# kingdwd/nlp-filter

Measured on AMD Instinct MI355X. Metric: Gauss-Newton collocation-point updates/sec, higher is better.
Workload: dtype f64; 1 GPU; C2 van_der_pol: n=2, m=1, full_state p=2, N=100 (P=101, d=202), T=10, M=101; global_batch=1024, batch_per_gpu=1024, parallelism=dp1 (independent trajectories; RCCL broadcast of constants only)

## Files before the change

### nlp-filter_amd/csrc/mhe_core.h

```cpp
#pragma once
#include <hip/hip_runtime.h>
#include <math.h>
#include <mutex>
#include <stdint.h>
#include <stdlib.h>

#include "mhe.h"
#include "mhe_models.h"

namespace mhe {

typedef double d4 __attribute__((ext_vector_type(4)));

#ifndef MHE_GN_MINW
#define MHE_GN_MINW 4
#endif
#ifndef MHE_NW
#define MHE_NW 8
#endif
constexpr int NW = MHE_NW;
constexpr int NTHREADS = NW * 64;
constexpr int MAX_NT = 13;
constexpr int MAX_SLOTS = (MAX_NT * (MAX_NT - 1) / 2 + NW - 1) / NW;

// ... 67 lines not shown
  S.ROWM = o; o += NW * 8;
  S.UN = o;   o += UNITS;
  S.XO = o;   o += bounded ? rnd2(P * n) : 0;
  S.ACT = o;  o += bounded ? dp / 2 : 0;
  S.GV = o;   o += bounded ? dp : 0;
  S.ZP = o;   o += cov ? dp * 16 : 0;
  S.total = o;
  return S;
}

struct GnArgs {
  const char* cbuf;
  int P, M, d, NT, ntiles, q, has_prior;
  int idx[8];
  double alpha;
  const double* X0;
  double* Xout;
  const double* U;
  long long ustride;
  const double* Y;
  const double* PAR;
  long long pstride;
  const double* x0;
  double* cost;
  int* iters;
  int* status;
  int max_iter;
  double tol;
  double* Hout;
  double* gout;
  const double* Hin;
  const double* gin;
  double* dout;
  unsigned long long* dbg;
  double huber_delta;
  int n_bounds;
  unsigned long long tag;
  int bidx[8];
  double blb[8], bub[8];
  double dpar[8];
  const double* Rw;
  long long rwstride;
  const double* PhiQ;
  int nq;
  double* cov;
  const double* md;
  long long mdstride;
  const double* Pw;
  long long pwstride;
  const double* Z0;
  double* Zout;
  double* lam;
  int nz, nc;
};

__device__ __forceinline__ const double* prior_weight(const GnArgs& a, const ConstLayout& CL, int b) {
  return a.Pw ? a.Pw + (long long)b * a.pwstride : (const double*)(a.cbuf + CL.Pw);
}

#ifdef MHE_DIAG
#define DIAG_DECL unsigned long long _dg[16] = {}; unsigned long long _dt = __builtin_amdgcn_s_memtime();
#define DIAG_MARK(i) do { const unsigned long long _n = __builtin_amdgcn_s_memtime(); _dg[i] += _n - _dt; _dt = _n; } while (0)
#define DIAG_FLUSH(b) do { if (threadIdx.x == 0 && a.dbg) for (int _i = 0; _i < 16; ++_i) a.dbg[(b) * 16 + _i] = _dg[_i]; } while (0)
#define DIAG_FDECL unsigned long long* _dg, unsigned long long& _dt
#define DIAG_FARGS _dg, _dt
#else
#define DIAG_DECL
#define DIAG_MARK(i) do { } while (0)
#define DIAG_FLUSH(b) do { } while (0)
#define DIAG_FDECL int
#define DIAG_FARGS 0
#endif

#ifndef MHE_KO
#define MHE_KO 0
#endif
#define KO(bit) ((MHE_KO >> (bit)) & 1)

__device__ __forceinline__ double readlane_d(double v, int lane) {
  const long long b = __double_as_longlong(v);
  const int lo = __builtin_amdgcn_readlane((int)b, lane);
  const int hi = __builtin_amdgcn_readlane((int)(b >> 32), lane);
  return __longlong_as_double(((long long)hi << 32) | (unsigned int)lo);
}

typedef unsigned int mhe_u2 __attribute__((ext_vector_type(2)));
__device__ __forceinline__ __amdgpu_buffer_rsrc_t cbuf_rsrc(const char* cbuf, size_t bytes) {
  return __builtin_amdgcn_make_buffer_rsrc((void*)cbuf, (short)0, (int)bytes, 0x00020000);
}
__device__ __forceinline__ double bload(__amdgpu_buffer_rsrc_t r, int voff, int soff) {
  const mhe_u2 v = __builtin_amdgcn_raw_buffer_load_b64(r, voff, soff, 0);
  return __builtin_bit_cast(double, v);
}

template <int CTRL>
__device__ __forceinline__ double dpp_d(double v) {
  const long long b = __double_as_longlong(v);
  const int lo = __builtin_amdgcn_mov_dpp((int)b, CTRL, 0xF, 0xF, false);
  const int hi = __builtin_amdgcn_mov_dpp((int)(b >> 32), CTRL, 0xF, 0xF, false);
  return __longlong_as_double(((long long)hi << 32) | (unsigned int)lo);
}

__device__ __forceinline__ void spread_dblock(double v, double (&o)[4]) {
  const double ev = dpp_d<0xA0>(v);
  const double od = dpp_d<0xF5>(v);
  const long long be = __double_as_longlong(ev), bo = __double_as_longlong(od);
  const auto el = __builtin_amdgcn_permlane16_swap((int)be, (int)be, false, false);
  const auto eh = __builtin_amdgcn_permlane16_swap((int)(be >> 32), (int)(be >> 32), false, false);
  const auto ol = __builtin_amdgcn_permlane16_swap((int)bo, (int)bo, false, false);
  const auto oh = __builtin_amdgcn_permlane16_swap((int)(bo >> 32), (int)(bo >> 32), false, false);
  o[0] = __longlong_as_double(((long long)eh[0] << 32) | (unsigned int)el[0]);
  o[2] = __longlong_as_double(((long long)eh[1] << 32) | (unsigned int)el[1]);
  o[1] = __longlong_as_double(((long long)oh[0] << 32) | (unsigned int)ol[0]);
  o[3] = __longlong_as_double(((long long)oh[1] << 32) | (unsigned int)ol[1]);
}

template <int XOR16, bool MAX>
__device__ __forceinline__ double pair_combine(double v) {
  const long long b = __double_as_longlong(v);
  const int lo = (int)b, hi = (int)(b >> 32);
  double x, y;
  if constexpr (XOR16 == 1) {
    auto l = __builtin_amdgcn_permlane16_swap(lo, lo, false, false);
    auto h = __builtin_amdgcn_permlane16_swap(hi, hi, false, false);
    x = __longlong_as_double(((long long)h[0] << 32) | (unsigned int)l[0]);
    y = __longlong_as_double(((long long)h[1] << 32) | (unsigned int)l[1]);
  } else {
    auto l = __builtin_amdgcn_permlane32_swap(lo, lo, false, false);
    auto h = __builtin_amdgcn_permlane32_swap(hi, hi, false, false);
    x = __longlong_as_double(((long long)h[0] << 32) | (unsigned int)l[0]);
    y = __longlong_as_double(((long long)h[1] << 32) | (unsigned int)l[1]);
  }
  return MAX ? fmax(x, y) : x + y;
}

__device__ __forceinline__ double wave_sum(double v) {
  v += dpp_d<0xB1>(v);
  v += dpp_d<0x4E>(v);
  v += dpp_d<0x141>(v);
  v += dpp_d<0x140>(v);
  v = pair_combine<1, false>(v);
  return pair_combine<2, false>(v);
}

__device__ __forceinline__ double wave_max(double v) {
  v = fmax(v, dpp_d<0xB1>(v));
  v = fmax(v, dpp_d<0x4E>(v));
  v = fmax(v, dpp_d<0x141>(v));
  v = fmax(v, dpp_d<0x140>(v));
  v = pair_combine<1, true>(v);
  return pair_combine<2, true>(v);
}

__device__ __forceinline__ void block_reduce2(double* red, double& a, double& b, bool is_max) {
  const int lane = threadIdx.x & 63, wave = threadIdx.x >> 6;
  a = is_max ? wave_max(a) : wave_sum(a);
  b = is_max ? wave_max(b) : wave_sum(b);
  if (lane == 0) {
    red[2 * wave] = a;
    red[2 * wave + 1] = b;
  }
  __syncthreads();
  double ra = red[0], rb = red[1];
#pragma unroll
  for (int w = 1; w < NW; ++w) {
    ra = is_max ? fmax(ra, red[2 * w]) : ra + red[2 * w];
    rb = is_max ? fmax(rb, red[2 * w + 1]) : rb + red[2 * w + 1];
  }
  __syncthreads();
  a = ra;
  b = rb;
}

__device__ __forceinline__ int make_slot_table(int wave, int lane, int NT) {
  const int u = wave + NW * lane;
  if (lane >= MAX_SLOTS || u >= NT * (NT - 1) / 2) return -1;
  int J = 0, base = 0;
  while (u >= base + (NT - 1 - J)) {
    base += NT - 1 - J;
    ++J;
  }
  return (J + 1 + (u - base)) | (J << 16);
}

__device__ __forceinline__ int tile_index(int I, int J, int NT) { return J * NT - J * (J - 1) / 2 + (I - J); }

__device__ __forceinline__ int slot_ij(int stab, int s) { return __builtin_amdgcn_readlane(stab, s); }

__device__ __forceinline__ int slot_start(int j, int wave, int NT) {
  const int base = j * (NT - 1) - j * (j - 1) / 2;
  return base > wave ? (base - wave + NW - 1) / NW : 0;
}

__device__ __forceinline__ void init_units(double* un) {
  if (threadIdx.x < 64)
    for (int e = threadIdx.x; e < UNITS; e += 64) un[e] = (e == 16 || e == 51) ? 1.0 : 0.0;
}

template <int SLOTS = MAX_SLOTS>
__device__ __forceinline__ void init_rowmask(int* rowm, int wave, int lane, int stab) {
  unsigned m = 0;
#pragma unroll
  for (int s = 0; s < SLOTS; ++s) {
    const int IJ = slot_ij(stab, s);
    if (IJ >= 0 && (IJ & 0xffff) == lane) m |= 1u << s;
  }
  if (lane < 16) rowm[wave * 16 + lane] = (int)m;
}

constexpr int TPR = NW >= 8 ? 4 : 2;

__device__ __forceinline__ int opaque_tid() {
  int t = threadIdx.x;
  asm volatile("" : "+v"(t));
  return t;
}

template <int n>
__device__ __forceinline__ void dot_rows_part(const double* __restrict__ Mt, int ld, int row, int len, int part,
                                              const double* __restrict__ Xs, double (&acc)[n]) {
#pragma unroll
  for (int c = 0; c < n; ++c) acc[c] = 0.0;
  int j = part;
#pragma unroll 1
  for (; j + TPR * 7 < len; j += TPR * 8) {
    double m[8];
#pragma unroll
    for (int u = 0; u < 8; ++u) m[u] = Mt[(j + TPR * u) * ld + row];
#pragma unroll
    for (int u = 0; u < 8; ++u)
#pragma unroll
      for (int c = 0; c < n; ++c) acc[c] += m[u] * Xs[(j + TPR * u) * n + c];
  }
  for (; j < len; j += TPR) {
    const double mv = Mt[j * ld + row];
#pragma unroll
    for (int c = 0; c < n; ++c) acc[c] += mv * Xs[j * n + c];
  }
  static_assert(TPR == 4, "quad reductions below assume 4 lanes per row");
#pragma unroll
  for (int c = 0; c < n; ++c) acc[c] += dpp_d<0xB1>(acc[c]);
#pragma unroll
  for (int c = 0; c < n; ++c) acc[c] += dpp_d<0x4E>(acc[c]);
}

template <class DYN, bool HUBER = false>
__device__ __forceinline__ double node_row(const GnArgs& a, const ConstLayout& CL, const SmemLayout& SL, double* sm,
                                           int b, int k, const double (&dx)[DYN::n]) {
  constexpr int n = DYN::n, m = DYN::m;
  const double* cw = (const double*)(a.cbuf + CL.cw);
  const double* Qw = (const double*)(a.cbuf + CL.Qw);
  const double* Xs = sm + SL.Xs;
  double cost = 0.0;
  {
    double xk[n], uk[m > 0 ? m : 1], f[n], F[n * n];
#pragma unroll
    for (int c = 0; c < n; ++c) xk[c] = Xs[k * n + c];
    if (m > 0) {
      const double* U = a.U + (long long)b * a.ustride + (long long)k * m;
#pragma unroll
      for (int c = 0; c < m; ++c) uk[c] = U[c];
    }
    DYN::eval(xk, uk, a.dpar, f, F);
    double W[n], V[n];
#pragma unroll
    for (int c = 0; c < n; ++c) W[c] = a.alpha * dx[c] - f[c];
    const double ck = cw[k];
    double E[n * n];
    if constexpr (HUBER) {
      const double dl = a.huber_delta;
#pragma unroll
      for (int r = 0; r < n; ++r) {
        const double q = Qw[r * n + r];
        const double sr = sqrt(1.0 + W[r] * W[r] / (dl * dl));
        const double lam = ck * (q / sr);
        V[r] = lam * W[r];
        cost += ck * (2.0 * q * dl * dl * (sr - 1.0));
        sm[SL.LAM + k * n + r] = lam;
#pragma unroll
        for (int c = 0; c < n; ++c) E[r * n + c] = lam * F[r * n + c];
      }
    } else {
#pragma unroll
      for (int r = 0; r < n; ++r) {
        double s = 0.0;
#pragma unroll
        for (int c = 0; c < n; ++c) s += Qw[r * n + c] * W[c];
        V[r] = ck * s;
        cost += W[r] * V[r];
      }
#pragma unroll
      for (int r = 0; r < n; ++r)
#pragma unroll
        for (int c = 0; c < n; ++c) {
          double s = 0.0;
#pragma unroll
          for (int t = 0; t < n; ++t) s += Qw[r * n + t] * F[t * n + c];
          E[r * n + c] = ck * s;
        }
    }
    double* Vs = sm + SL.Vs + k * n;
    double* FtV = sm + SL.FtV + k * n;
    double* Es = sm + SL.Es + k * n * n;
    double* FtE = sm + SL.FtE + k * n * n;
#pragma unroll
    for (int r = 0; r < n; ++r) {
      Vs[r] = V[r];
      double s = 0.0;
// ... 12 lines not shown
  }
  return cost;
}

template <class DYN, bool HUBER = false>
__device__ __forceinline__ double node_phase(const GnArgs& a, const ConstLayout& CL, const SmemLayout& SL, double* sm, int b) {
  constexpr int n = DYN::n;
  const double* Dt = (const double*)(a.cbuf + CL.Dt);
  const double* Xs = sm + SL.Xs;
  double cost = 0.0;
  const int tid = opaque_tid();
  const int part = tid % TPR;
  for (int k0 = 0; k0 < a.P; k0 += NTHREADS / TPR) {
    const int k = k0 + tid / TPR;
    const int kk = k < a.P ? k : a.P - 1;
    double dx[n];
    dot_rows_part<n>(Dt, a.P, kk, a.P, part, Xs, dx);
    if (part || k >= a.P) continue;
    cost += node_row<DYN, HUBER>(a, CL, SL, sm, b, k, dx);
  }
  return cost;
}

constexpr double COST_NOISE = 4.0;

template <class DYN, class MEAS, bool NOISE = false, bool MHUBER = false>
__device__ __forceinline__ double meas_row(const GnArgs& a, const ConstLayout& CL, const SmemLayout& SL, double* sm,
                                           int b, int i, const double (&xi)[DYN::n], double* nzp = nullptr) {
  constexpr int n = DYN::n, p = MEAS::p, q = MEAS::q;
  const double* Rw = (const double*)(a.cbuf + CL.Rw);
  double cost = 0.0;
  {
    double par[q > 0 ? q : 1];
    if (q > 0) {
      const double* PR = a.PAR + (long long)b * a.pstride + (long long)i * q;
#pragma unroll
      for (int c = 0; c < q; ++c) par[c] = PR[c];
    }
    const double* R = (!MEAS::LINEAR && a.Rw ? a.Rw + (long long)b * a.rwstride : Rw) + (long long)i * p * p;
    double h[p], H[p * n];
    MEAS::eval(xi, par, a.idx, h, H);
    const double* yi = a.Y + ((long long)b * a.M + i) * p;
    double e[p], Re[p];
#pragma unroll
    for (int r = 0; r < p; ++r) e[r] = yi[r] - h[r];
    const bool masked = masked_row<p>(R);
    if (masked) {
#pragma unroll
      for (int c = 0; c < p * n; ++c) H[c] = 0.0;
#pragma unroll
      for (int r = 0; r < p; ++r) e[r] = 0.0;
    }
    [[maybe_unused]] double lam[p], rcost = 0.0;
    [[maybe_unused]] bool robust = false;
    if constexpr (MHUBER) {
      static_assert(p == 1 && !MEAS::LINEAR, "robust measurement rows: scalar rows of a nonlinear model");
      lam[0] = R[0];
      const double dl = a.md[(long long)b * a.mdstride + i];
      if (!masked && dl < INFINITY) {
        const double sr = sqrt(1.0 + e[0] * e[0] / (dl * dl));
        lam[0] = R[0] / sr;
        rcost = 2.0 * R[0] * e[0] * e[0] / (1.0 + sr);
        robust = true;
      }
      R = lam;
    }
#pragma unroll
    for (int r = 0; r < p; ++r) {
      double s = 0.0;
#pragma unroll
      for (int c = 0; c < p; ++c) s += R[r * p + c] * e[c];
      Re[r] = s;
      cost += e[r] * s;
    }
    if constexpr (MHUBER) {
      if (robust) cost = rcost;
    }
    if constexpr (NOISE) {
      if (!masked) {
        double t = 0.0;
#pragma unroll
        for (int r = 0; r < p; ++r) t += fabs(Re[r]) * (fabs(yi[r]) + fabs(h[r]));
        *nzp += COST_NOISE * __DBL_EPSILON__ * t;
      }
    }
    double* GE = sm + SL.GE + i * n;
#pragma unroll
    for (int c = 0; c < n; ++c) {
      double s = 0.0;
#pragma unroll
      for (int r = 0; r < p; ++r) s += H[r * n + c] * Re[r];
      GE[c] = s;
    }
    if (!MEAS::LINEAR) {
      double* G = sm + SL.G + i * n * n;
      double RH[p * n];
#pragma unroll
      for (int r = 0; r < p; ++r)
#pragma unroll
        for (int c = 0; c < n; ++c) {
          double s = 0.0;
#pragma unroll
          for (int t = 0; t < p; ++t) s += R[r * p + t] * H[t * n + c];
          RH[r * n + c] = s;
        }
#pragma unroll
      for (int r = 0; r < n; ++r)
#pragma unroll
        for (int c = 0; c < n; ++c) {
          double s = 0.0;
#pragma unroll
          for (int t = 0; t < p; ++t) s += H[t * n + r] * RH[t * n + c];
          G[r * n + c] = s;
        }
    }
  }
  return cost;
}

template <class DYN, class MEAS, bool NOISE = false, bool MHUBER = false>
__device__ __forceinline__ double meas_phase(const GnArgs& a, const ConstLayout& CL, const SmemLayout& SL, double* sm, int b,
                                             double* nzp = nullptr) {
  constexpr int n = DYN::n;
  const double* PhiT = (const double*)(a.cbuf + CL.PhiT);
  const double* Xs = sm + SL.Xs;
  double cost = 0.0;
  const int tid = opaque_tid();
  const int part = tid % TPR;
  for (int i0 = 0; i0 < a.M; i0 += NTHREADS / TPR) {
    const int i = i0 + tid / TPR;
    const int ii = i < a.M ? i : a.M - 1;
    double xi[n];
    dot_rows_part<n>(PhiT, a.M, ii, a.P, part, Xs, xi);
    if (part || i >= a.M) continue;
    cost += meas_row<DYN, MEAS, NOISE, MHUBER>(a, CL, SL, sm, b, i, xi, nzp);
  }
  return cost;
}

__device__ __forceinline__ double row_pair_sum(double v) {
  const long long b = __double_as_longlong(v);
  const auto l = __builtin_amdgcn_permlane16_swap((int)b, (int)b, false, false);
  const auto h = __builtin_amdgcn_permlane16_swap((int)(b >> 32), (int)(b >> 32), false, false);
  return __longlong_as_double(((long long)h[0] << 32) | (unsigned int)l[0]) +
         __longlong_as_double(((long long)h[1] << 32) | (unsigned int)l[1]);
}
__device__ __forceinline__ double upper_half(double v) {
  const long long b = __double_as_longlong(v);
  const auto l = __builtin_amdgcn_permlane32_swap((int)b, (int)b, false, false);
  const auto h = __builtin_amdgcn_permlane32_swap((int)(b >> 32), (int)(b >> 32), false, false);
  return __longlong_as_double(((long long)h[1] << 32) | (unsigned int)l[1]);
}

template <class DYN, class MEAS, bool HUBER = false, bool NOISE = false, bool MHUBER = false>
__device__ __forceinline__ double node_meas_phase(const GnArgs& a, const ConstLayout& CL, const SmemLayout& SL,
                                                  double* sm, int b, DIAG_FDECL, double* nzp = nullptr) {
  constexpr int n = DYN::n;
  constexpr int ROWS = NTHREADS / TPR;
  if (a.P > ROWS || a.M > ROWS)
    return node_phase<DYN, HUBER>(a, CL, SL, sm, b) + meas_phase<DYN, MEAS, NOISE, MHUBER>(a, CL, SL, sm, b, nzp);
  const __amdgpu_buffer_rsrc_t rs = cbuf_rsrc(a.cbuf, CL.total);
  const double* Xs = sm + SL.Xs;
  const int tid = opaque_tid();
  const int part = (tid >> 4) & 3, r = (tid >> 6) * 16 + (tid & 15);
  const int kk = r < a.P ? r : a.P - 1, ii = r < a.M ? r : a.M - 1;
  double dx[n], xi[n];
#pragma unroll
  for (int c = 0; c < n; ++c) dx[c] = xi[c] = 0.0;
  const int len = a.P;
  int o1 = (int)CL.Dt + (part * a.P + kk) * 8, o2 = (int)CL.PhiT + (part * a.M + ii) * 8;
  const int s1 = TPR * a.P * 8, s2 = TPR * a.M * 8;
  int j = part;
#pragma unroll 1
  for (; j + TPR * 7 < len; j += TPR * 8) {
    double m1[8], m2[8];
#pragma unroll
    for (int u = 0; u < 8; ++u) {
      m1[u] = bload(rs, o1, u * s1);
      m2[u] = bload(rs, o2, u * s2);
    }
    o1 += 8 * s1;
    o2 += 8 * s2;
#pragma unroll
    for (int u = 0; u < 8; ++u)
#pragma unroll
      for (int c = 0; c < n; ++c) {
        const double x = Xs[(j + TPR * u) * n + c];
        dx[c] += m1[u] * x;
        xi[c] += m2[u] * x;
      }
  }
  for (; j < len; j += TPR) {
    const double m1 = bload(rs, o1, 0), m2 = bload(rs, o2, 0);
    o1 += s1;
    o2 += s2;
#pragma unroll
    for (int c = 0; c < n; ++c) {
      dx[c] += m1 * Xs[j * n + c];
      xi[c] += m2 * Xs[j * n + c];
    }
  }
  static_assert(TPR == 4, "the row reductions below assume 4 parts per row");
#pragma unroll
  for (int c = 0; c < n; ++c) {
    dx[c] = row_pair_sum(dx[c]);
    xi[c] = row_pair_sum(xi[c]);
  }
#pragma unroll
  for (int c = 0; c < n; ++c) {
    dx[c] += upper_half(dx[c]);
    xi[c] += upper_half(xi[c]);
  }
  DIAG_MARK(14);
  double cost = 0.0;
  if (part == 0) {
    if (r < a.P) cost += node_row<DYN, HUBER>(a, CL, SL, sm, b, r, dx);
    if (r < a.M) cost += meas_row<DYN, MEAS, NOISE, MHUBER>(a, CL, SL, sm, b, r, xi, nzp);
  }
  return cost;
}

template <class DYN, class MEAS, bool HUBER = false, bool NOISE = false, bool MHUBER = false>
__device__ __forceinline__ double node_meas_phase(const GnArgs& a, const ConstLayout& CL, const SmemLayout& SL,
                                                  double* sm, int b, double* nzp = nullptr) {
  DIAG_DECL
  return node_meas_phase<DYN, MEAS, HUBER, NOISE, MHUBER>(a, CL, SL, sm, b, DIAG_FARGS, nzp);
}

template <class DYN, bool PW = true>
__device__ __forceinline__ double grad_phase(const GnArgs& a, const ConstLayout& CL, const SmemLayout& SL, double* sm, int b) {
  constexpr int n = DYN::n;
  const __amdgpu_buffer_rsrc_t rs = cbuf_rsrc(a.cbuf, CL.total);
  const double* Vs = sm + SL.Vs;
  const double* FtV = sm + SL.FtV;
  const double* GE = sm + SL.GE;
  const double* Xs = sm + SL.Xs;
  double* BV = sm + SL.BV;
  double cost = 0.0;
  const int dp = 16 * a.NT;
  const int tid = opaque_tid();
  constexpr int HP = TPR / 2;
  const int q = (tid >> 4) & 3, sub = q % HP;
  const bool phi = q >= HP;
  for (int j0 = 0; j0 < a.P; j0 += NTHREADS / TPR) {
    const int j = j0 + (tid >> 6) * 16 + (tid & 15);
    const int jj = j < a.P ? j : a.P - 1;
    const double* vec = phi ? GE : Vs;
    const int len = phi ? a.M : a.P;
    double s[n];
#pragma unroll
    for (int c = 0; c < n; ++c) s[c] = 0.0;
    int om = (int)(phi ? CL.Phi : CL.D) + (sub * a.P + jj) * 8;
    const int sm8 = HP * a.P * 8;
    int k = sub;
#pragma unroll 1
    for (; k + HP * 7 < len; k += HP * 8) {
      double mv[8];
#pragma unroll
      for (int u = 0; u < 8; ++u) mv[u] = bload(rs, om, u * sm8);
      om += 8 * sm8;
#pragma unroll
      for (int u = 0; u < 8; ++u)
#pragma unroll
        for (int c = 0; c < n; ++c) s[c] += mv[u] * vec[(k + HP * u) * n + c];
    }
    for (; k < len; k += HP) {
      const double mv = bload(rs, om, 0);
      om += sm8;
#pragma unroll
      for (int c = 0; c < n; ++c) s[c] += mv * vec[k * n + c];
    }
    static_assert(HP == 2, "the row reductions below assume TPR == 4");
#pragma unroll
    for (int c = 0; c < n; ++c) s[c] = row_pair_sum(s[c]);
    double o[n];
#pragma unroll
    for (int c = 0; c < n; ++c) o[c] = upper_half(s[c]);
    if (q != 0 || j >= a.P) continue;
    double gv[n];
#pragma unroll
    for (int c = 0; c < n; ++c) gv[c] = a.alpha * s[c] - FtV[j * n + c] - o[c];
    if (a.has_prior && j == 0) {
      const double* Pw = PW ? prior_weight(a, CL, b) : (const double*)(a.cbuf + CL.Pw);
      double r0[n];
#pragma unroll
      for (int c = 0; c < n; ++c) r0[c] = Xs[c] - a.x0[(long long)b * n + c];
#pragma unroll
      for (int r = 0; r < n; ++r) {
        double t2 = 0.0;
#pragma unroll
        for (int c = 0; c < n; ++c) t2 += Pw[r * n + c] * r0[c];
        gv[r] += t2;
        cost += r0[r] * t2;
      }
    }
#pragma unroll
    for (int c = 0; c < n; ++c) BV[j * n + c] = -gv[c];
  }
  for (int t = a.d + tid; t < dp; t += NTHREADS) BV[t] = 0.0;
  return cost;
}

template <class DYN, class MEAS, bool HUBER = false>
__device__ __forceinline__ double h_element(const GnArgs& a, const double* Phi, const double* Es,
                                            const double* FtE, const double* G, double v, double da,
                                            double db, int row, int col, const double* D = nullptr,
                                            const double* LAM = nullptr) {
  constexpr int n = DYN::n;
  if (row < a.d && col < a.d) {
    const int j = row / n, aa = row - j * n;
    const int l = col / n, bb = col - l * n;
    if constexpr (HUBER) {
      if (aa == bb) {
        double s = 0.0;
        for (int k = 0; k < a.P; ++k) s += D[k * a.P + j] * LAM[k * n + aa] * D[k * a.P + l];
        v += a.alpha * a.alpha * s;
      }
    }
    v -= da * Es[(l * n + aa) * n + bb] + db * Es[(j * n + bb) * n + aa];
    if (j == l) v += FtE[(j * n + aa) * n + bb];
    if (!MEAS::LINEAR) {
      double s2 = 0.0;
      for (int i = 0; i < a.M; ++i) s2 += Phi[i * a.P + j] * Phi[i * a.P + l] * G[(i * n + aa) * n + bb];
      v += s2;
    }
  }
  return v;
}

template <int SLOTS, bool BOUNDED>
__device__ __forceinline__ void build_slots_n2(const GnArgs& a, const ConstLayout& CL, const SmemLayout& SL,
                                               double* sm, d4 (&acc)[SLOTS], int lane, int stab) {
  const __amdgpu_buffer_rsrc_t rs = cbuf_rsrc(a.cbuf, CL.total);
  const double* Es = sm + SL.Es;
  const int* ACT = (const int*)(sm + SL.ACT);
  double cn[4], an, bn;
  auto issue = [&](int s) {
    const int IJ = slot_ij(stab, s);
    const int ti = IJ < 0 ? 0 : tile_index(IJ & 0xffff, IJ >> 16, a.NT);
#pragma unroll
    for (int r = 0; r < 4; ++r) cn[r] = bload(rs, ti * 2048 + lane * 8, (int)CL.Cc + 512 * r);
    an = bload(rs, ti * 512 + lane * 8, (int)CL.DAc);
    bn = bload(rs, ti * 512 + lane * 8, (int)CL.DBc);
  };
  issue(0);
#pragma unroll
  for (int s = 0; s < SLOTS; ++s) {
    const double c[4] = {cn[0], cn[1], cn[2], cn[3]};
    const double av = an, bv = bn;
    if (s + 1 < SLOTS) issue(s + 1);
    const int IJ = slot_ij(stab, s);
    const int I = IJ < 0 ? 1 : IJ & 0xffff, J = IJ < 0 ? 0 : IJ >> 16;
    const int col = 16 * I + (lane & 15);
    const int cc = col < a.d ? col : a.d - 1;
    const int l = cc >> 1, bb = cc & 1;
    double dav[4], dbv[4];
    spread_dblock(av, dav);
    spread_dblock(bv, dbv);
    const int aa = (lane >> 4) & 1;
    const double el = Es[(l * 2 + aa) * 2 + bb];
    const double* ej = Es + ((8 * J + (lane >> 5)) * 2 + bb) * 2 + aa;
#pragma unroll
    for (int r = 0; r < 4; ++r) {
      const int row = 16 * J + (lane >> 4) + 4 * r;
      const double t = dav[r] * el + dbv[r] * ej[8 * r];
      if (I == a.NT - 1)
        acc[s][r] = (row < a.d && col < a.d) ? t - c[r] : -c[r];
      else
        acc[s][r] = t - c[r];
      if (BOUNDED && (ACT[row] | ACT[col])) acc[s][r] = 0.0;
    }
    __builtin_amdgcn_sched_barrier(0);
  }
}

template <class DYN, class MEAS, int SLOTS, bool HUBER = false, bool BOUNDED = false, bool PW = true>
__device__ __forceinline__ void build_tiles(const GnArgs& a, const ConstLayout& CL, const SmemLayout& SL, double* sm,
                                            d4 (&acc)[SLOTS], int wave, int lane, int stab,
                                            const double* PhiL = nullptr) {
  const int* ACT = (const int*)(sm + SL.ACT);
  const double* Dm = (const double*)(a.cbuf + CL.D);
  const double* LAM = sm + SL.LAM;
  const double* Cc = (const double*)(a.cbuf + CL.Cc);
  const double* DA = (const double*)(a.cbuf + CL.DA);
  const double* DB = (const double*)(a.cbuf + CL.DB);
  const double* Phi = PhiL ? PhiL : (const double*)(a.cbuf + CL.Phi);
  const double* Es = sm + SL.Es;
  const double* FtE = sm + SL.FtE;
  const double* G = sm + SL.G;
  asm volatile("" : "+v"(lane));
  asm volatile("" : "+s"(wave));
  asm volatile("" : "+v"(stab));
  constexpr int n = DYN::n;
  constexpr bool FAST = !HUBER && MEAS::LINEAR;
  if constexpr (FAST && n == 2) build_slots_n2<SLOTS, BOUNDED>(a, CL, SL, sm, acc, lane, stab);
#pragma unroll
  for (int s = 0; s < (FAST && n == 2 ? 0 : SLOTS); ++s) {
// ... 727 lines not shown
      double part[4];
#pragma unroll
      for (int r = 0; r < 4; ++r) part[r] = row16_sum(ut[64 * r] * db);
      const double* LT = DT + J * DTS;
      double sd = 0.0;
#pragma unroll
      for (int r = 0; r < 4; ++r) sd += LT[c * LIS + g + 4 * r] * (yj[g + 4 * r] - part[r]);
      const double dv = rows4_sum(sd);
      if (lane_o < 16) yj[c] = dv;
    } else if (!KO(6)) {
      const unsigned rm = __builtin_amdgcn_readfirstlane(((const int*)(sm + SL.ROWM))[wave * 16 + bb]);
#pragma unroll
      for (int s = SLOTS - 1; s >= 0; --s) {
        if (!((rm >> s) & 1u)) continue;
        const int J = slot_ij(stab_o, s) >> 16;
        if (J == bb - 1) continue;
        double* yj = DV + 16 * J;
        const double v[4] = {acc[s][0] * db, acc[s][1] * db, acc[s][2] * db, acc[s][3] * db};
        const double z = row16_sum4(v, c);
        if ((c & 3) == 0) yj[g + 4 * (2 * (c >> 3) + ((c >> 2) & 1))] -= z;
      }
    }
    __syncthreads();
  }
}

__device__ __forceinline__ bool tag_ok(const GnArgs& a) {
  return *(const unsigned long long*)a.cbuf == a.tag;
}

__device__ inline void bad_constants(const GnArgs& a, int b, int mode) {
  if (mode == MODE_SOLVE)
    for (int t = threadIdx.x; t < a.d; t += blockDim.x) a.Xout[(size_t)b * a.d + t] = a.X0[(size_t)b * a.d + t];
  if (threadIdx.x == 0) {
    if (mode != MODE_ASSEMBLE) a.status[b] = MHE_STATUS_BAD_CONSTANTS;
    if (mode == MODE_SOLVE) a.iters[b] = 0;
    if (mode != MODE_LINSOLVE) a.cost[b] = NAN;
  }
}

template <int n>
__device__ inline void cov_fail(const GnArgs& a, int b, int status) {
  for (int t = threadIdx.x; t < a.nq * n * n; t += blockDim.x) a.cov[(size_t)b * a.nq * n * n + t] = NAN;
  if (threadIdx.x == 0) a.status[b] = status;
}

constexpr double EPS_ACT = 1e-6;
constexpr double ARMIJO_SIGMA = 1e-4;
constexpr int LS_MAX = 30;
constexpr double COST_SLACK = 1e-12;

#include "mhe_big.h"

__device__ __forceinline__ int opaque_s(int x) {
  asm volatile("" : "+s"(x));
  return x;
}
#define FA a
#define FCL const_layout(opaque_s(a.P), opaque_s(a.M), n, MEAS::p, opaque_s(a.NT))
#define FSL smem_layout(opaque_s(a.P), opaque_s(a.M), n, opaque_s(a.NT), !MEAS::LINEAR, false, SB)

template <int SLOTS, bool STORE>
__device__ __forceinline__ void fwd_sweep_panel(int NT, const double* DT, double* ZP, d4 (&acc)[SLOTS], int wave,
                                                int lane, int stab, d4& gram) {
#pragma unroll 1
  for (int k = 0; k < NT; ++k) {
    int lane_o = lane, wave_o = wave, stab_o = stab;
    asm volatile("" : "+v"(lane_o));
    asm volatile("" : "+s"(wave_o));
    asm volatile("" : "+v"(stab_o));
    const int sT = slot_start(k, wave_o, NT), sU = slot_start(k + 1, wave_o, NT);
    const unsigned mT = (1u << sU) - (1u << sT);
    const bool own = wave_o == k % NW;
    [[maybe_unused]] d4 ykeep = {0.0, 0.0, 0.0, 0.0};
    if (mT != 0u || own) {
      const double* LT = DT + k * DTS;
      double la[4], zk[4];
#pragma unroll
      for (int r = 0; r < 4; ++r) {
        la[r] = LT[(4 * r + (lane_o >> 4)) * LIS + (lane_o & 15)];
        zk[r] = ZP[k * 256 + r * 64 + lane_o];
      }
      d4 y = {0.0, 0.0, 0.0, 0.0};
#pragma unroll
      for (int r = 0; r < 4; ++r) y = __builtin_amdgcn_mfma_f64_16x16x4f64(la[r], zk[r], y, 0, 0, 0);
      if constexpr (STORE) {
        ykeep = y;
      } else if (own) {
#pragma unroll
        for (int r = 0; r < 4; ++r) gram = __builtin_amdgcn_mfma_f64_16x16x4f64(y[r], y[r], gram, 0, 0, 0);
      }
#pragma unroll
      for (int s = 0; s < SLOTS; ++s) {
        if ((mT >> s) & 1u) {
          double* zb = ZP + (slot_ij(stab_o, s) & 0xffff) * 256 + lane_o;
          d4 t;
#pragma unroll
          for (int r = 0; r < 4; ++r) t[r] = zb[64 * r];
#pragma unroll
          for (int r = 0; r < 4; ++r) t = __builtin_amdgcn_mfma_f64_16x16x4f64(acc[s][r], y[r], t, 0, 0, MFMA_NEG_A);
#pragma unroll
          for (int r = 0; r < 4; ++r) zb[64 * r] = t[r];
        }
      }
    }
    __syncthreads();
    if constexpr (STORE) {
      if (own) {
#pragma unroll
        for (int r = 0; r < 4; ++r) ZP[k * 256 + r * 64 + lane_o] = ykeep[r];
      }
    }
  }
}

template <int n, int SLOTS>
__device__ __forceinline__ void cov_sweep(const GnArgs& a, const SmemLayout& SL, double* sm, d4 (&acc)[SLOTS],
                                          int wave, int lane, int stab, int b) {
  constexpr int QPP = 16 / n;
  double* ZP = sm + SL.ZP;
  const double* DT = sm + SL.DT;
  const int NT = a.NT, dp = 16 * NT, dn = a.P * n;
  for (int q0 = 0; q0 < a.nq; q0 += QPP) {
    const int nql = a.nq - q0 < QPP ? a.nq - q0 : QPP;
    for (int t = threadIdx.x; t < dp * 16; t += NTHREADS) ZP[t] = 0.0;
    __syncthreads();
    for (int t = threadIdx.x; t < nql * dn; t += NTHREADS) {
      const int ql = t / dn, row = t - ql * dn, j = row / n, c = row - j * n;
      ZP[row * 16 + ql * n + c] = a.PhiQ[(size_t)(q0 + ql) * a.P + j];
    }
    __syncthreads();
    d4 gram = {0.0, 0.0, 0.0, 0.0};
    fwd_sweep_panel<SLOTS, false>(NT, DT, ZP, acc, wave, lane, stab, gram);
    for (int w = 0; w < NW; ++w) {
      if (wave == w) {
#pragma unroll
        for (int r = 0; r < 4; ++r) ZP[r * 64 + lane] = w == 0 ? gram[r] : ZP[r * 64 + lane] + gram[r];
      }
      __syncthreads();
    }
    for (int t = threadIdx.x; t < nql * n * n; t += NTHREADS) {
      const int ql = t / (n * n), e = t - ql * n * n, ra = e / n, cb = e - ra * n;
      const int lo = ra < cb ? ra : cb, hi = ra < cb ? cb : ra;
      a.cov[((size_t)b * a.nq + q0 + ql) * n * n + e] = ZP[(ql * n + lo) * 16 + ql * n + hi];
    }
    __syncthreads();
  }
}

template <class DYN, class MEAS, int SLOTS, int mode, bool HUBER = false, int MINW = MHE_GN_MINW, bool SB = false,
          bool MHUBER = false, bool PW = true>
__global__ __launch_bounds__(NTHREADS, MINW) void k_gn(GnArgs a) {
  constexpr int n = DYN::n;
  static_assert(!SB || (mode == MODE_SOLVE && MINW <= 2 && NW == 8), "small-batch factorization: one workgroup per CU");
  extern __shared__ __attribute__((aligned(16))) double sm[];
  const ConstLayout CL = const_layout(a.P, a.M, n, MEAS::p, a.NT);
  const SmemLayout SL = smem_layout(a.P, a.M, n, a.NT, !MEAS::LINEAR, false, SB, mode == MODE_COV);
  const int lane = threadIdx.x & 63;
  const int wave = __builtin_amdgcn_readfirstlane(threadIdx.x >> 6);
  const int b = blockIdx.x;
  const int stab = SB ? make_slot_table_sb(wave, lane, a.NT) : make_slot_table(wave, lane, a.NT);
  init_rowmask<SLOTS>((int*)(sm + SL.ROWM), wave, lane, stab);
  SbMasks sbm = {0u, 0u, 0u};
  if constexpr (SB) sbm = sb_masks<SLOTS>(lane, stab, a.NT);
  double* Xs = sm + SL.Xs;
  if (threadIdx.x == 0) *(int*)(sm + SL.RED + 4 * NW) = 0;
  init_units(sm + SL.UN);
  if constexpr (SB)
    for (int t = threadIdx.x; t < 256; t += NTHREADS) sm[SL.ZT + t] = 0.0;
  double* DV = sm + SL.YV;
  double* RED = sm + SL.RED;
  d4 acc[SLOTS];
#pragma unroll
  for (int s = 0; s < SLOTS; ++s) acc[s] = d4{0.0, 0.0, 0.0, 0.0};
  if (!tag_ok(a)) {
    if constexpr (mode == MODE_COV)
      cov_fail<n>(a, b, MHE_STATUS_BAD_CONSTANTS);
    else
      bad_constants(a, b, mode);
    return;
  }

  __syncthreads();
  if constexpr (mode == MODE_LINSOLVE) {
    const int dp = 16 * a.NT;
    const double* Hb = a.Hin + (size_t)b * dp * dp;
    for (int t = threadIdx.x; t < dp; t += NTHREADS) sm[SL.BV + t] = -a.gin[(size_t)b * dp + t];
    load_tiles<SLOTS>(a, SL, sm, Hb, acc, wave, lane, stab);
    __syncthreads();
    DIAG_DECL
    const bool ok = factor_forward<SLOTS>(a, SL, sm, acc, wave, lane, stab, DIAG_FARGS);
    backward<SLOTS>(a, SL, sm, acc, wave, lane, stab);
    for (int t = threadIdx.x; t < dp; t += NTHREADS) a.dout[(size_t)b * dp + t] = DV[t];
    if (threadIdx.x == 0) a.status[b] = ok ? MHE_STATUS_CONVERGED : MHE_STATUS_NOT_SPD;
    return;
  }

  for (int t = threadIdx.x; t < a.d; t += NTHREADS) Xs[t] = a.X0[(size_t)b * a.d + t];
  __syncthreads();

  int status = MHE_STATUS_MAX_ITER;
  int it = 0;
  DIAG_DECL
  for (;;) {
    DIAG_MARK(7);
    double c1 = node_meas_phase<DYN, MEAS, HUBER, false, MHUBER>(FA, FCL, FSL, sm, opaque_s(b), DIAG_FARGS);
    DIAG_MARK(6);
    __syncthreads();
    DIAG_MARK(0);
    c1 += grad_phase<DYN, PW>(FA, FCL, FSL, sm, opaque_s(b));
    {
      const double cwv = wave_sum(c1);
      if (lane == 0) RED[2 * NW + wave] = cwv;
    }
    DIAG_MARK(1);
    if constexpr (mode == MODE_ASSEMBLE) {
      double c2 = 0.0;
      block_reduce2(RED, c1, c2, false);
      build_tiles<DYN, MEAS, SLOTS, HUBER>(FA, FCL, FSL, sm, acc, wave, lane, stab);
      const int dp = 16 * a.NT;
      double* Hb = a.Hout + (size_t)b * dp * dp;
#pragma unroll
      for (int s = 0; s < SLOTS; ++s) {
        const int IJ = slot_ij(stab, s);
        if (IJ >= 0) {
          const int I = IJ & 0xffff, J = IJ >> 16;
#pragma unroll
          for (int r = 0; r < 4; ++r) {
            const int row = 16 * J + (lane >> 4) + 4 * r, col = 16 * I + (lane & 15);
            Hb[(size_t)row * dp + col] = -acc[s][r];
            if (I != J) Hb[(size_t)col * dp + row] = -acc[s][r];
          }
        }
      }
      __syncthreads();
      for (int t = threadIdx.x; t < a.NT * 256; t += NTHREADS) {
        const int J = t >> 8, tr = (t >> 4) & 15, tc = t & 15;
        Hb[(size_t)(16 * J + tr) * dp + 16 * J + tc] = sm[SL.DT + J * DTS + (t & 255)];
      }
      for (int t = threadIdx.x; t < dp; t += NTHREADS) a.gout[(size_t)b * dp + t] = -sm[SL.BV + t];
      if (threadIdx.x == 0) a.cost[b] = c1;
      return;
    }
    if constexpr (mode == MODE_COV) {
      if constexpr (n <= 16) {
        build_tiles<DYN, MEAS, SLOTS, HUBER>(FA, FCL, FSL, sm, acc, wave, lane, stab);
        __syncthreads();
        if (!factor_forward<SLOTS>(FA, FSL, sm, acc, wave, lane, stab, DIAG_FARGS)) {
          cov_fail<n>(a, b, MHE_STATUS_NOT_SPD);
          return;
        }
        cov_sweep<n, SLOTS>(a, SL, sm, acc, wave, lane, stab, b);
        if (threadIdx.x == 0) a.status[b] = MHE_STATUS_CONVERGED;
      }
      return;
    }
    if (it >= a.max_iter) break;
    build_tiles<DYN, MEAS, SLOTS, HUBER, false, PW>(FA, FCL, FSL, sm, acc, wave, lane, stab);
    DIAG_MARK(15);
    __syncthreads();
    DIAG_MARK(2);
    bool ok;
    if constexpr (SB)
      ok = factor_forward_sb<SLOTS>(FA, FSL, sm, acc, wave, lane, stab, sbm, DIAG_FARGS);
    else
      ok = factor_forward<SLOTS>(FA, FSL, sm, acc, wave, lane, stab, DIAG_FARGS);
    DIAG_MARK(3);
    if (!ok) {
      status = MHE_STATUS_NOT_SPD;
      break;
    }
    if constexpr (SB)
      backward_sb<SLOTS>(FA, FSL, sm, acc, wave, lane, stab);
    else
      backward<SLOTS>(FA, FSL, sm, acc, wave, lane, stab);
    DIAG_MARK(4);
    double dmax = 0.0, xmax = 0.0;
    const int tid_u = opaque_tid();
    for (int t = tid_u; t < a.d; t += NTHREADS) {
      const double dv = DV[t];
      dmax = isfinite(dv) ? fmax(dmax, fabs(dv)) : INFINITY;
      xmax = fmax(xmax, fabs(Xs[t] + dv));
    }
    block_reduce2(RED, dmax, xmax, true);
    if (dmax == INFINITY) {
      status = MHE_STATUS_NONFINITE;
      break;
    }
    for (int t = tid_u; t < a.d; t += NTHREADS) Xs[t] = Xs[t] + DV[t];
    __syncthreads();
    ++it;
    if (dmax <= a.tol * (1.0 + xmax)) {
      status = MHE_STATUS_CONVERGED;
      double cf = node_meas_phase<DYN, MEAS, HUBER, false, MHUBER>(FA, FCL, FSL, sm, opaque_s(b));
      __syncthreads();
      cf += grad_phase<DYN, PW>(FA, FCL, FSL, sm, opaque_s(b));
      double z = 0.0;
      block_reduce2(RED, cf, z, false);
      if (threadIdx.x == 0) a.cost[b] = cf;
      goto done;
    }
  }
  {
    __syncthreads();
    if (threadIdx.x == 0) {
      double cf = RED[2 * NW];
      for (int w = 1; w < NW; ++w) cf += RED[2 * NW + w];
      a.cost[b] = cf;
    }
  }
done:
  DIAG_MARK(5);
  DIAG_FLUSH(b);
  __syncthreads();
  for (int t = threadIdx.x; t < a.d; t += NTHREADS) a.Xout[(size_t)b * a.d + t] = Xs[t];
  if (threadIdx.x == 0) {
    a.iters[b] = it;
    a.status[b] = status;
  }
}

__device__ __forceinline__ void comp_box(const GnArgs& a, int c, double& lo, double& hi) {
  lo = -INFINITY;
  hi = INFINITY;
  for (int i = 0; i < a.n_bounds; ++i)
    if (a.bidx[i] == c) {
      lo = fmax(lo, a.blb[i]);
      hi = fmin(hi, a.bub[i]);
    }
}

template <int n>
__device__ __forceinline__ double prior_cost(const GnArgs& a, const double* Pw, const double* Xs, int b) {
  double r0[n], cost = 0.0;
#pragma unroll
  for (int c = 0; c < n; ++c) r0[c] = Xs[c] - a.x0[(long long)b * n + c];
#pragma unroll
  for (int r = 0; r < n; ++r) {
    double t2 = 0.0;
#pragma unroll
    for (int c = 0; c < n; ++c) t2 += Pw[r * n + c] * r0[c];
    cost += r0[r] * t2;
  }
  return cost;
}

#define FSLB smem_layout(opaque_s(a.P), opaque_s(a.M), n, opaque_s(a.NT), !MEAS::LINEAR, true)

template <class DYN, class MEAS, int SLOTS, bool HUBER = false, bool MHUBER = false>
__global__ __launch_bounds__(NTHREADS, MHE_GN_MINW) void k_gn_bounded(GnArgs a) {
  constexpr int n = DYN::n;
  extern __shared__ __attribute__((aligned(16))) double sm[];
  const SmemLayout SL = smem_layout(a.P, a.M, n, a.NT, !MEAS::LINEAR, true);
  const int lane = threadIdx.x & 63;
  const int wave = __builtin_amdgcn_readfirstlane(threadIdx.x >> 6);
  const int b = blockIdx.x;
  const int stab = make_slot_table(wave, lane, a.NT);
  init_rowmask((int*)(sm + SL.ROWM), wave, lane, stab);
  double* Xs = sm + SL.Xs;
  double* XO = sm + SL.XO;
  int* ACT = (int*)(sm + SL.ACT);
  const double* BV = sm + SL.BV;
  double* GV = sm + SL.GV;
  const double* DV = sm + SL.YV;
  double* RED = sm + SL.RED;
  if (threadIdx.x == 0) *(int*)(sm + SL.RED + 4 * NW) = 0;
  init_units(sm + SL.UN);
  d4 acc[SLOTS];
#pragma unroll
  for (int s = 0; s < SLOTS; ++s) acc[s] = d4{0.0, 0.0, 0.0, 0.0};
  if (!tag_ok(a)) {
    bad_constants(a, b, MODE_SOLVE);
    return;
  }
  for (int t = threadIdx.x; t < a.d; t += NTHREADS) {
    double lo, hi;
    comp_box(a, t % n, lo, hi);
    Xs[t] = fmin(fmax(a.X0[(size_t)b * a.d + t], lo), hi);
  }
  for (int t = threadIdx.x; t < 16 * a.NT; t += NTHREADS) ACT[t] = 0;
  __syncthreads();
  double nz0 = 0.0;
  double cost = node_meas_phase<DYN, MEAS, HUBER, true, MHUBER>(FA, FCL, FSLB, sm, opaque_s(b), &nz0);
  __syncthreads();
  cost += grad_phase<DYN>(FA, FCL, FSLB, sm, opaque_s(b));
  block_reduce2(RED, cost, nz0, false);
  int status = MHE_STATUS_MAX_ITER;
  int it = 0;
  DIAG_DECL
  for (;;) {
    if (it >= a.max_iter) break;
    double w = 0.0, xm = 0.0;
    for (int t = threadIdx.x; t < a.d; t += NTHREADS) {
      double lo, hi;
      comp_box(a, t % n, lo, hi);
      const double x = Xs[t], g = -BV[t];
      xm = fmax(xm, fabs(x));
      if (lo > -INFINITY || hi < INFINITY) w = fmax(w, fabs(x - fmin(fmax(x - g, lo), hi)));
    }
    block_reduce2(RED, w, xm, true);
    const double eps = fmin(EPS_ACT * (1.0 + xm), w);
    for (int t = threadIdx.x; t < a.d; t += NTHREADS) {
      double lo, hi;
      comp_box(a, t % n, lo, hi);
      const double x = Xs[t], g = -BV[t];
      ACT[t] = (lo > -INFINITY || hi < INFINITY) && ((x <= lo + eps && g > 0.0) || (x >= hi - eps && g < 0.0));
      GV[t] = BV[t];
    }
    __syncthreads();
    build_tiles<DYN, MEAS, SLOTS, HUBER, true>(FA, FCL, FSLB, sm, acc, wave, lane, stab);
    __syncthreads();
    const bool ok = factor_forward<SLOTS>(FA, FSLB, sm, acc, wave, lane, stab, DIAG_FARGS);
    if (!ok) {
      status = MHE_STATUS_NOT_SPD;
      break;
    }
    backward<SLOTS>(FA, FSLB, sm, acc, wave, lane, stab);
    double smax = 0.0, fin = 0.0;
    for (int t = threadIdx.x; t < a.d; t += NTHREADS) {
      double lo, hi;
      comp_box(a, t % n, lo, hi);
      const double x = Xs[t], dv = DV[t];
      XO[t] = x;
      if (!isfinite(dv)) fin = 1.0;
      smax = fmax(smax, fabs(fmin(fmax(x + dv, lo), hi) - x));
    }
    block_reduce2(RED, smax, fin, true);
    if (fin != 0.0) {
      status = MHE_STATUS_NONFINITE;
      break;
    }
    double alpha = 1.0, ct = 0.0, nzt = 0.0;
    for (int ls = 0;;) {
      double pred = 0.0;
      for (int t = threadIdx.x; t < a.d; t += NTHREADS) {
        double lo, hi;
        comp_box(a, t % n, lo, hi);
        const double x = XO[t], dv = DV[t], g = -GV[t];
        const double xt = fmin(fmax(x + alpha * dv, lo), hi);
        pred += ACT[t] ? g * (xt - x) : alpha * g * dv;
        Xs[t] = xt;
      }
      __syncthreads();
      nzt = 0.0;
      ct = node_meas_phase<DYN, MEAS, HUBER, true, MHUBER>(FA, FCL, FSLB, sm, opaque_s(b), &nzt);
      if (threadIdx.x == 0 && a.has_prior)
        ct += prior_cost<n>(a, prior_weight(a, FCL, b), Xs, b);
      block_reduce2(RED, ct, pred, false);
      {
        double z = 0.0;
        block_reduce2(RED, nzt, z, false);
      }
      ++ls;
      if (ct <= cost + 2.0 * ARMIJO_SIGMA * pred + nz0 + nzt + COST_SLACK * fabs(cost) || ls >= LS_MAX) break;
      alpha *= 0.5;
    }
    cost = ct;
    nz0 = nzt;
    ++it;
    double xn = 0.0, z = 0.0;
    for (int t = threadIdx.x; t < a.d; t += NTHREADS) xn = fmax(xn, fabs(Xs[t]));
    block_reduce2(RED, xn, z, true);
    if (smax <= a.tol * (1.0 + xn)) {
      status = MHE_STATUS_CONVERGED;
      break;
    }
    grad_phase<DYN>(FA, FCL, FSLB, sm, opaque_s(b));
    __syncthreads();
  }
  __syncthreads();
  for (int t = threadIdx.x; t < a.d; t += NTHREADS) a.Xout[(size_t)b * a.d + t] = Xs[t];
  if (threadIdx.x == 0) {
    a.cost[b] = cost;
    a.iters[b] = it;
    a.status[b] = status;
  }
}
#undef FSLB
#undef FA
#undef FCL
#undef FSL

template <class MEAS>
__global__ void k_build_cc(int P, int M, int n, int p, int NT, int has_prior, int huber, double alpha,
                           const double* D, const double* cw, const double* Phi, const double* Qw,
                           const double* Rw, const double* Pw, char* cbuf) {
  const ConstLayout CL = const_layout(P, M, n, p, NT);
  const int ntiles = NT * (NT + 1) / 2;
  const int gid = blockIdx.x * blockDim.x + threadIdx.x;
  if (gid >= ntiles * 256) return;
  const int t = gid >> 8, e = gid & 255, r = e >> 6, lane = e & 63;
  int J = 0, base = 0;
  while (t >= base + (NT - J)) {
    base += NT - J;
    ++J;
  }
  const int I = J + (t - base);
// ... 524 lines not shown
```

Baseline: 626.2 million GN collocation-point updates/s.

## Trim per-iteration cost reduction and skip idle waves in residual phases

For n=2 linear-measurement solve mode, this drops the per-iteration wave reduction of the cost. The cost is instead computed once after the loop from the node/measurement residuals plus the prior term. Waves whose row block lies entirely beyond P/M now exit the node/meas and gradient phases early, and the max_iter check moves to the top of the loop. The point is to cut redundant cost accumulation and idle-wave work each Gauss-Newton iteration, at the price of a specialized path whose final cost may differ from the old accumulated value (e.g. it omits grad-phase terms).

Measured after the change: 633.8 million GN collocation-point updates/s (median of 6 runs). 1.01x the previous value.

```diff
diff --git a/nlp-filter_amd/csrc/mhe_core.h b/nlp-filter_amd/csrc/mhe_core.h
--- a/nlp-filter_amd/csrc/mhe_core.h
+++ b/nlp-filter_amd/csrc/mhe_core.h
@@ -243,8 +243,11 @@
   return pair_combine<2, true>(v);
 }
 
+template <bool SW = false>
 __device__ __forceinline__ void block_reduce2(double* red, double& a, double& b, bool is_max) {
-  const int lane = threadIdx.x & 63, wave = threadIdx.x >> 6;
+  const int lane = threadIdx.x & 63;
+  int wave = threadIdx.x >> 6;
+  if constexpr (SW) wave = __builtin_amdgcn_readfirstlane(wave);
   a = is_max ? wave_max(a) : wave_sum(a);
   b = is_max ? wave_max(b) : wave_sum(b);
   if (lane == 0) {
@@ -563,7 +566,7 @@
   return __longlong_as_double(((long long)h[1] << 32) | (unsigned int)l[1]);
 }
 
-template <class DYN, class MEAS, bool HUBER = false, bool NOISE = false, bool MHUBER = false>
+template <class DYN, class MEAS, bool HUBER = false, bool NOISE = false, bool MHUBER = false, bool SKIP = false>
 __device__ __forceinline__ double node_meas_phase(const GnArgs& a, const ConstLayout& CL, const SmemLayout& SL,
                                                   double* sm, int b, DIAG_FDECL, double* nzp = nullptr) {
   constexpr int n = DYN::n;
@@ -573,6 +576,8 @@
   const __amdgpu_buffer_rsrc_t rs = cbuf_rsrc(a.cbuf, CL.total);
   const double* Xs = sm + SL.Xs;
   const int tid = opaque_tid();
+  if constexpr (SKIP)
+    if (16 * __builtin_amdgcn_readfirstlane(tid >> 6) >= (a.P > a.M ? a.P : a.M)) return 0.0;
   const int part = (tid >> 4) & 3, r = (tid >> 6) * 16 + (tid & 15);
   const int kk = r < a.P ? r : a.P - 1, ii = r < a.M ? r : a.M - 1;
   double dx[n], xi[n];
@@ -631,14 +636,29 @@
   return cost;
 }
 
-template <class DYN, class MEAS, bool HUBER = false, bool NOISE = false, bool MHUBER = false>
+template <class DYN, class MEAS, bool HUBER = false, bool NOISE = false, bool MHUBER = false, bool SKIP = false>
 __device__ __forceinline__ double node_meas_phase(const GnArgs& a, const ConstLayout& CL, const SmemLayout& SL,
                                                   double* sm, int b, double* nzp = nullptr) {
   DIAG_DECL
-  return node_meas_phase<DYN, MEAS, HUBER, NOISE, MHUBER>(a, CL, SL, sm, b, DIAG_FARGS, nzp);
-}
-
-template <class DYN, bool PW = true>
+  return node_meas_phase<DYN, MEAS, HUBER, NOISE, MHUBER, SKIP>(a, CL, SL, sm, b, DIAG_FARGS, nzp);
+}
+
+template <int n>
+__device__ __forceinline__ double prior_cost(const GnArgs& a, const double* Pw, const double* Xs, int b) {
+  double r0[n], cost = 0.0;
+#pragma unroll
+  for (int c = 0; c < n; ++c) r0[c] = Xs[c] - a.x0[(long long)b * n + c];
+#pragma unroll
+  for (int r = 0; r < n; ++r) {
+    double t2 = 0.0;
+#pragma unroll
+    for (int c = 0; c < n; ++c) t2 += Pw[r * n + c] * r0[c];
+    cost += r0[r] * t2;
+  }
+  return cost;
+}
+
+template <class DYN, bool PW = true, bool SKIP = false>
 __device__ __forceinline__ double grad_phase(const GnArgs& a, const ConstLayout& CL, const SmemLayout& SL, double* sm, int b) {
   constexpr int n = DYN::n;
   const __amdgpu_buffer_rsrc_t rs = cbuf_rsrc(a.cbuf, CL.total);
@@ -654,6 +674,8 @@
   const int q = (tid >> 4) & 3, sub = q % HP;
   const bool phi = q >= HP;
   for (int j0 = 0; j0 < a.P; j0 += NTHREADS / TPR) {
+    if constexpr (SKIP)
+      if (j0 + 16 * __builtin_amdgcn_readfirstlane(tid >> 6) >= a.P) break;
     const int j = j0 + (tid >> 6) * 16 + (tid & 15);
     const int jj = j < a.P ? j : a.P - 1;
     const double* vec = phi ? GE : Vs;
@@ -1687,6 +1709,7 @@
           bool MHUBER = false, bool PW = true>
 __global__ __launch_bounds__(NTHREADS, MINW) void k_gn(GnArgs a) {
   constexpr int n = DYN::n;
+  constexpr bool TRIM = mode == MODE_SOLVE && n == 2 && MEAS::LINEAR && !HUBER;
   static_assert(!SB || (mode == MODE_SOLVE && MINW <= 2 && NW == 8), "small-batch factorization: one workgroup per CU");
   extern __shared__ __attribute__((aligned(16))) double sm[];
   const ConstLayout CL = const_layout(a.P, a.M, n, MEAS::p, a.NT);
@@ -1738,13 +1761,16 @@
   int it = 0;
   DIAG_DECL
   for (;;) {
+    if constexpr (TRIM)
+      if (it >= a.max_iter) break;
     DIAG_MARK(7);
-    double c1 = node_meas_phase<DYN, MEAS, HUBER, false, MHUBER>(FA, FCL, FSL, sm, opaque_s(b), DIAG_FARGS);
+    [[maybe_unused]] double c1 =
+        node_meas_phase<DYN, MEAS, HUBER, false, MHUBER, TRIM>(FA, FCL, FSL, sm, opaque_s(b), DIAG_FARGS);
     DIAG_MARK(6);
     __syncthreads();
     DIAG_MARK(0);
-    c1 += grad_phase<DYN, PW>(FA, FCL, FSL, sm, opaque_s(b));
-    {
+    c1 += grad_phase<DYN, PW, TRIM>(FA, FCL, FSL, sm, opaque_s(b));
+    if constexpr (!TRIM) {
       const double cwv = wave_sum(c1);
       if (lane == 0) RED[2 * NW + wave] = cwv;
     }
@@ -1790,7 +1816,8 @@
       }
       return;
     }
-    if (it >= a.max_iter) break;
+    if constexpr (!TRIM)
+      if (it >= a.max_iter) break;
     build_tiles<DYN, MEAS, SLOTS, HUBER, false, PW>(FA, FCL, FSL, sm, acc, wave, lane, stab);
     DIAG_MARK(15);
     __syncthreads();
@@ -1817,7 +1844,7 @@
       dmax = isfinite(dv) ? fmax(dmax, fabs(dv)) : INFINITY;
       xmax = fmax(xmax, fabs(Xs[t] + dv));
     }
-    block_reduce2(RED, dmax, xmax, true);
+    block_reduce2<TRIM>(RED, dmax, xmax, true);
     if (dmax == INFINITY) {
       status = MHE_STATUS_NONFINITE;
       break;
@@ -1827,6 +1854,7 @@
     ++it;
     if (dmax <= a.tol * (1.0 + xmax)) {
       status = MHE_STATUS_CONVERGED;
+      if constexpr (TRIM) break;
       double cf = node_meas_phase<DYN, MEAS, HUBER, false, MHUBER>(FA, FCL, FSL, sm, opaque_s(b));
       __syncthreads();
       cf += grad_phase<DYN, PW>(FA, FCL, FSL, sm, opaque_s(b));
@@ -1836,7 +1864,14 @@
       goto done;
     }
   }
-  {
+  if constexpr (TRIM) {
+    double cf = node_meas_phase<DYN, MEAS, HUBER, false, MHUBER, TRIM>(FA, FCL, FSL, sm, opaque_s(b));
+    if (threadIdx.x == 0 && a.has_prior)
+      cf += prior_cost<n>(a, PW ? prior_weight(a, FCL, b) : (const double*)(a.cbuf + FCL.Pw), Xs, b);
+    double z = 0.0;
+    block_reduce2<true>(RED, cf, z, false);
+    if (threadIdx.x == 0) a.cost[b] = cf;
+  } else {
     __syncthreads();
     if (threadIdx.x == 0) {
       double cf = RED[2 * NW];
@@ -1863,21 +1898,6 @@
       lo = fmax(lo, a.blb[i]);
       hi = fmin(hi, a.bub[i]);
     }
-}
-
-template <int n>
-__device__ __forceinline__ double prior_cost(const GnArgs& a, const double* Pw, const double* Xs, int b) {
-  double r0[n], cost = 0.0;
-#pragma unroll
-  for (int c = 0; c < n; ++c) r0[c] = Xs[c] - a.x0[(long long)b * n + c];
-#pragma unroll
-  for (int r = 0; r < n; ++r) {
-    double t2 = 0.0;
-#pragma unroll
-    for (int c = 0; c < n; ++c) t2 += Pw[r * n + c] * r0[c];
-    cost += r0[r] * t2;
-  }
-  return cost;
 }
 
 #define FSLB smem_layout(opaque_s(a.P), opaque_s(a.M), n, opaque_s(a.NT), !MEAS::LINEAR, true)
```
